# zfkuang/PaletteNeRF

Hardware: AMD Instinct MI355X
Metric: rendered_samples_per_sec (higher is better)
Workload: dtype f32 (field: f16x3 split products, fp32 accumulate); 1 GPU; configs[1]: NeRF-synthetic lego geometry (scene S0), -m nerf inference, 800x800, 1 view(s)/step, camera moving (one pose of the path per step); march_mode=native, fused_field=True, field_precision=f16x3, half_tables=False, ray_order=tile8, frames_in_flight=1, gathered_floats_per_ray=0, rccl_ranks=1, parallelism=single GPU

## Files before the change

### palettenerf_amd/csrc/frame.hip

```cpp
#include "pnr_common.hpp"
#include "march_core.hpp"
#include "grid_core.hpp"
#include "field_core.hpp"
#include "frame_plan.hpp"
#include <hip/hip_ext.h>
#include <vector>
#include <stdlib.h>

uint64_t pnr_internal_edit_device_bytes();
int pnr_internal_edit_upload(const pnr_palette_edit* edit, void* dst, hipStream_t s);
int pnr_internal_palette_field_forward(const pnr_palette_field_args* a, pnr_stream_t stream, int waves12);

#ifndef PNR_FRAME_LEVEL_PAIRS
#define PNR_FRAME_LEVEL_PAIRS 1
#endif
#ifndef PNR_FRAME_LEVEL_PAIRS_PAL
#define PNR_FRAME_LEVEL_PAIRS_PAL 0
#endif
namespace pnr {

struct FrameCtl {
    int32_t n_alive, n_step, step, done;
    int32_t iterations, pad0;
    unsigned long long rendered;
// ... 537 lines not shown
        typedef uint32_t RowT __attribute__((ext_vector_type(NW)));
        __half acc[2 * NT];
#pragma unroll
        for (int ch = 0; ch < 2 * NT; ch++) acc[ch] = __float2half(0.0f);
        if (grid_corner_rows<1>(g, lc, b, idxs, pos)) {
            RowT v[8];
            gather8<RowT, 1, ORDERED>(static_cast<const RowT*>(table) + lc.off0, idxs, v);
            grid_corner_weights(pos, ws);
#pragma unroll
            for (uint32_t idx = 0; idx < 8; idx++) {
                __half hv[2 * NT];
                __builtin_memcpy(hv, &v[idx], sizeof(hv));
#pragma unroll
                for (int ch = 0; ch < 2 * NT; ch++)
                    acc[ch] = __float2half(__half2float(acc[ch]) + __half2float(__float2half(ws[idx] * __half2float(hv[ch]))));
            }
        }
        *reinterpret_cast<float2*>(enc0 + o) = make_float2(__half2float(acc[0]), __half2float(acc[1]));
        if constexpr (NT >= 2) *reinterpret_cast<float2*>(g.enc[1] + o) = make_float2(__half2float(acc[2]), __half2float(acc[3]));
        if constexpr (NT == 3) *reinterpret_cast<float2*>(g.enc[2] + o) = make_float2(__half2float(acc[4]), __half2float(acc[5]));
    }
}

#ifdef PNR_HOSTED_TIMING
__device__ unsigned long long g_hosted_timing[8 + 8 * 256 + 2 * 16 * 128];
__device__ int g_hosted_timing_iter = 3;
#endif
#ifndef PNR_HOSTED_MIN_GLOG
#define PNR_HOSTED_MIN_GLOG 3u
#endif
#ifndef PNR_HOSTED_JUMPS
#define PNR_HOSTED_JUMPS false
#endif
template <int KIND>
__device__ __forceinline__ void hosted_march_tail(const FrameCtl* ctl, const GridArgs& g, const HostedArgs& ha) {
    struct { uint32_t blocks; const int32_t* qctr; const StragglerRec* qrecs; const float* rays_o; const float* rays_d; const uint8_t* bitfield;
             const uint32_t* mip; MarchParams p; float* xyzs; float* dirs; float* deltas; int32_t* partials; } h;
    {
        const HostedConst* hc = ha.hc;
        const int par = ctl->iterations & 1;
        h.blocks = ha.blocks; h.qctr = hc->qctr_all + par * kQueueCtrs; h.qrecs = hc->qrecs; h.rays_o = hc->rays_o; h.rays_d = hc->rays_d;
        h.bitfield = hc->bitfield; h.mip = hc->mip; h.p = hc->p; h.xyzs = hc->xyzs; h.dirs = hc->dirs; h.deltas = hc->deltas;
        h.partials = hc->partials[par] + ha.partial_base;
    }
    __builtin_amdgcn_s_setprio(3);
    __shared__ float lv_scale[16];
// ... 80 lines not shown
            for (uint32_t pi = (uint32_t)lane; pi < cnt * 16u; pi += PNR_WAVE) {
                const uint32_t b = wrows[wave][pi >> 4], level = pi & 15u;
                LevelCtx lc;
                lc.scale = lv_scale[level]; lc.resolution = lv_res[level]; lc.off0 = lv_off[level]; lc.hashmap_size = lv_size[level];
                lc.kind = 0u;
                for (uint32_t tz = 0; tz < n_tab; tz++) grid_row<KIND, false>(g, lc, level, g.table[tz], g.enc[tz], b);
            }
            wave_lds_sync();
        }
    }
    for (int off = PNR_WAVE / 2; off > 0; off >>= 1) emitted += __shfl_xor(emitted, off, PNR_WAVE);
    if (lane == 0) wemit[wave] = emitted;
    __syncthreads();
    if (threadIdx.x == 0) {
        uint32_t tot = 0;
        for (int wv = 0; wv < (int)(kRayBlock / PNR_WAVE); wv++) tot += wemit[wv];
        h.partials[blockIdx.x] = (int32_t)tot;
#ifdef PNR_HOSTED_TIMING
        if (timing) tm[3] = wall_clock64();
#endif
    }
}

template <int KIND>
__device__ __forceinline__ void frame_grid_body(const FrameCtl* __restrict__ ctl, const GridArgs& g, const HostedArgs& h) {
    if (ctl->done) return;
    constexpr uint32_t kLv = KIND == GK_SINGLE ? (PNR_FRAME_LEVEL_PAIRS == 2 ? 4u : (PNR_FRAME_LEVEL_PAIRS ? 2u : 1u))
                                               : ((KIND == GK_PAIR && PNR_FRAME_LEVEL_PAIRS_PAL) ? 2u : 1u);
    constexpr bool kPairs = kLv > 1;
    constexpr uint32_t kNY = 16u / kLv;
    uint32_t bx = blockIdx.x, by = blockIdx.y, bz = blockIdx.z, nbx = gridDim.x;
    if (h.blocks) {
        if (bx < h.blocks) {
#ifndef PNR_NO_HOSTED_CODE
            hosted_march_tail<KIND>(ctl, g, h);
#endif
            return;
        }
        const uint32_t id = bx - h.blocks, yz = id / h.gx;
        bx = id - yz * h.gx; by = yz % kNY; bz = yz / kNY; nbx = h.gx;
    }
    const uint32_t stride = nbx * 256u;
    const uint32_t rows = (uint32_t)ctl->n_alive * (uint32_t)ctl->n_step;
    const uint32_t level = 15u - by;
#ifdef PNR_HOSTED_TIMING
    const bool timing = ctl->iterations == g_hosted_timing_iter && (bx & 15u) == 0 && bx < 2048u && bz == 0;
    unsigned long long* tmm = g_hosted_timing + 8 + 8 * 256 + 2 * (level * 128 + (bx >> 4));
    if (timing && threadIdx.x == 0) tmm[0] = wall_clock64();
#endif
    const LevelCtx lc = level_ctx(g, level);
    [[maybe_unused]] const LevelCtx lc2 = level_ctx(g, kPairs ? by : level);
    [[maybe_unused]] const LevelCtx lc3 = level_ctx(g, kLv == 4 ? 11u - by : level), lc4 = level_ctx(g, kLv == 4 ? 4u + by : level);
    const void* table = g.table[KIND == GK_SINGLE ? bz : 0];
    float* enc0 = g.enc[KIND == GK_SINGLE ? bz : 0];
    for (uint32_t b = bx * 256u + threadIdx.x; b < rows; b += stride) {
        const float d0 = g.deltas[(size_t)b * 2];
        const uint32_t fl = h.rowflag ? h.rowflag[b] : 0u;
        if (d0 == 0.0f || fl) continue;
        grid_row<KIND>(g, lc, level, table, enc0, b);
        if constexpr (kLv == 4) { grid_row<KIND>(g, lc3, 11u - by, table, enc0, b); grid_row<KIND>(g, lc4, 4u + by, table, enc0, b); }
        if constexpr (kPairs) grid_row<KIND>(g, lc2, by, table, enc0, b);
    }
#ifdef PNR_HOSTED_TIMING
    if (timing && threadIdx.x == 0) { asm volatile("s_waitcnt vmcnt(0)" ::: "memory"); tmm[1] = wall_clock64(); }
#endif
}

#ifndef PNR_GRID_WAVES
#define PNR_GRID_WAVES 8
#endif
#ifndef PNR_GRID_WAVES_SINGLE
#define PNR_GRID_WAVES_SINGLE 7
#endif
#define PNR_GRID_KERNEL(NAME, KIND, WAVES)                                                                                                   \
    __global__ void __launch_bounds__(256) __attribute__((amdgpu_waves_per_eu(WAVES))) NAME(const FrameCtl* __restrict__ ctl, GridArgs g, HostedArgs h) { \
        frame_grid_body<KIND>(ctl, g, h);                                                                                                    \
    }
PNR_GRID_KERNEL(k_frame_grid, GK_SINGLE, PNR_GRID_WAVES_SINGLE)
PNR_GRID_KERNEL(k_frame_grid_pair, GK_PAIR, PNR_GRID_WAVES)
PNR_GRID_KERNEL(k_frame_grid_triple, GK_TRIPLE, PNR_GRID_WAVES)
PNR_GRID_KERNEL(k_frame_grid_h1, GK_HALF1, PNR_GRID_WAVES)
PNR_GRID_KERNEL(k_frame_grid_h2, GK_HALF2, PNR_GRID_WAVES)
PNR_GRID_KERNEL(k_frame_grid_h3, GK_HALF3, PNR_GRID_WAVES)
#undef PNR_GRID_KERNEL

__global__ void __launch_bounds__(256) k_interleave_tables(const float2* __restrict__ a, const float2* __restrict__ b, uint64_t rows,
                                                           float4* __restrict__ out) {
    const uint64_t i = (uint64_t)blockIdx.x * 256 + threadIdx.x;
    if (i < rows) { const float2 u = a[i], v = b[i]; out[i] = make_float4(u.x, u.y, v.x, v.y); }
}
__global__ void __launch_bounds__(256) k_interleave_tables3(const float2* __restrict__ a, const float2* __restrict__ b, const float2* __restrict__ c,
                                                            uint64_t rows, float4* __restrict__ out) {
    const uint64_t i = (uint64_t)blockIdx.x * 256 + threadIdx.x;
    if (i < rows) {
        const float2 u = a[i], v = b[i], t = c[i];
        out[2 * i] = make_float4(u.x, u.y, v.x, v.y);
        out[2 * i + 1] = make_float4(t.x, t.y, 0.0f, 0.0f);
    }
}
__global__ void __launch_bounds__(256) k_interleave_tables3_half(const float2* __restrict__ a, const float2* __restrict__ b, const float2* __restrict__ c,
                                                                 uint64_t rows, uint4* __restrict__ out) {
// ... 251 lines not shown
    w.partials[1] = reinterpret_cast<int32_t*>(take((kMaxMarchBlocks + kHostedBlocks) * 4));
    w.enc_pal = w.enc_clip = w.aux = nullptr;
    w.edit = nullptr;
    if (aux_stride) {
        w.edit = take(pnr_internal_edit_device_bytes());
        w.enc_pal = reinterpret_cast<float*>(take(n * 16 * 2 * 4));
        if (with_clip) w.enc_clip = reinterpret_cast<float*>(take(n * 16 * 2 * 4));
        w.aux = reinterpret_cast<float*>(take(n * aux_stride * 4));
    }
    w.s_o = reinterpret_cast<float*>(take(n * 12)); w.s_d = reinterpret_cast<float*>(take(n * 12));
    w.s_noise = reinterpret_cast<float*>(take(n * 4)); w.s_far = reinterpret_cast<float*>(take(n * 4));
    w.s_ws = reinterpret_cast<float*>(take(n * 4)); w.s_depth = reinterpret_cast<float*>(take(n * 4));
    w.s_image = reinterpret_cast<float*>(take(n * 12));
    w.s_aux = aux_stride ? reinterpret_cast<float*>(take(n * aux_stride * 4)) : nullptr;
    w.hosted = reinterpret_cast<HostedConst*>(take(sizeof(HostedConst)));
    w.qctr = reinterpret_cast<int32_t*>(take(2 * kQueueCtrs * 4));
    w.qrecs = reinterpret_cast<StragglerRec*>(take(n * sizeof(StragglerRec)));
    w.rowflag = reinterpret_cast<uint8_t*>(take(n));
    w.bytes = off;
    return w;
}

struct FrameOpts {
    int aux_fusion, composite_fusion, hosted_tail, dynamic_tiles, march_budget, march_budget0, march_blocks, iteration_margin, block_skip, coop_march, palette_waves12;
};
static FrameOpts frame_opts_now() {
    return FrameOpts{g_opt_aux_fusion, g_opt_composite_fusion, g_opt_hosted_tail, g_opt_dynamic_tiles, g_opt_march_budget, g_opt_march_budget0, g_opt_march_blocks,
                     g_opt_iteration_margin, g_opt_block_skip, g_opt_coop_march, g_opt_palette_waves12};
}

using UnsortKernel = decltype(&k_frame_unsort_outputs<4>);
using MarchKernel = decltype(&k_frame_march<true, true, 1>);
using GridKernel = decltype(&k_frame_grid);
using FieldKernel = decltype(&k_frame_field<0, false>);

struct FramePlan {
    pnr_stream_t stream; const void* workspace;
    uint32_t N, max_steps, aux_stride, n_enc, march_lds;
    float T_thresh, density_scale, enc_scale;
    FrameWorkspace w;
    const float *in_o, *in_d, *in_far, *noise_p;
    float *out_ws, *out_depth, *out_image, *out_aux;
    const int32_t* ray_order;
    float *ray_ws, *ray_depth, *ray_image, *ray_aux;
    const uint8_t* bitfield; const uint32_t* mip; const float* packed_weights;
    bool with_clip, half_tables, hosted, use_mip, pow2, pal_composite_fused, timing, has_edit;
    int aux_fused;
    int composite_fused;
    MarchParams mp;
    GridArgs ga;
    pnr_palette_field_args pf;
// ... 77 lines not shown
    p.bitfield = a->bitfield; p.mip = static_cast<const uint32_t*>(a->mip); p.packed_weights = a->packed_weights;
    p.stats = a->stats; p.kernel_ms = a->kernel_ms; p.timing = a->kernel_ms != nullptr;

    p.n_enc = pal ? (p.with_clip ? 3u : 2u) : 1u;
    p.aux_fused = (pal && opt.aux_fusion && pnr_palette_field_stages_aux(pal->num_basis, pal->clip_dim, pal->pred_clip)) ? 1 : 0;
    p.composite_fused = (!pal && opt.composite_fusion) ? opt.composite_fusion : 0;
    p.pal_composite_fused = pal && p.aux_fused && opt.composite_fusion == 2;
    p.half_tables = a->table_dtype == PNR_DTYPE_F16;
    if (p.half_tables && pal && (p.with_clip ? !pal->embeddings_triple : !pal->embeddings_pair)) return PNR_ERR_UNSUPPORTED;
    if (a->table_dtype != PNR_DTYPE_F32 && a->table_dtype != PNR_DTYPE_F16) return PNR_ERR_UNSUPPORTED;

    GridArgs& ga = p.ga;
    ga.xyzs = w.xyzs; ga.deltas = w.deltas; ga.offsets = a->offsets; ga.lp = make_level_params(16, a->S, a->base_resolution); ga.level_stride = p.N;
    ga.bound = a->bound; ga.two_bound = 2.0f * a->bound; ga.inv_two_bound = exact_reciprocal_or_zero(ga.two_bound);
    ga.gridtype = a->gridtype;
    ga.enc[0] = w.enc; ga.enc[1] = w.enc_pal; ga.enc[2] = w.enc_clip;
    p.lookup_y = 16; p.lookup_z = 1;
    if (p.half_tables && pal && p.with_clip) { p.lookup = k_frame_grid_h3; ga.table[0] = pal->embeddings_triple; }
    else if (p.half_tables && pal) { p.lookup = k_frame_grid_h2; ga.table[0] = pal->embeddings_pair; }
    else if (p.half_tables) { p.lookup = k_frame_grid_h1; ga.table[0] = a->embeddings; }
    else if (pal && p.with_clip && pal->embeddings_triple) { p.lookup = k_frame_grid_triple; ga.table[0] = pal->embeddings_triple; }
    else if (pal && !p.with_clip && pal->embeddings_pair) { p.lookup = k_frame_grid_pair; ga.table[0] = pal->embeddings_pair; p.lookup_y = PNR_FRAME_LEVEL_PAIRS_PAL ? 8 : 16; }
    else {
        p.lookup = k_frame_grid; p.lookup_y = PNR_FRAME_LEVEL_PAIRS == 2 ? 4 : (PNR_FRAME_LEVEL_PAIRS ? 8 : 16); p.lookup_z = p.n_enc;
        ga.table[0] = a->embeddings; ga.table[1] = pal ? pal->embeddings_palette : nullptr; ga.table[2] = p.with_clip ? pal->embeddings_clip : nullptr;
    }

    if (pal) {
        pnr_palette_field_args& pf = p.pf;
        pf.enc = w.enc; pf.enc_palette = w.enc_pal; pf.enc_clip = w.enc_clip; pf.level_stride = p.N; pf.dirs = w.dirs; pf.deltas = w.deltas;
        pf.packed = a->packed_weights; pf.num_basis = pal->num_basis;
        pf.clip_dim = pal->clip_dim; pf.pred_clip = pal->pred_clip; pf.density_scale = a->density_scale; pf.offsets_weight = pal->offsets_weight;
        pf.view_dep_weight = pal->view_dep_weight; pf.aux_stride = p.aux_stride; pf.sigmas = w.sigmas; pf.rgbs = w.rgbs; pf.aux = w.aux;
        pf.precision = a->field_precision; pf.xyzs = w.xyzs;
        for (int k = 0; k < 3; k++) pf.enc_scale[k] = a->enc_scale[k];
        pf.overflow_flag = a->watch_overflow ? w.scratch + 1 : nullptr;
        pf.tile_counter = opt.dynamic_tiles ? w.scratch + 2 : nullptr;
        if (p.aux_fused) { pf.weights_sum = p.out_ws; pf.aux_map = p.out_aux; pf.T_thresh = a->T_thresh; }
        if (p.pal_composite_fused) { pf.rays_t = w.rays_t; pf.weights_sum_rw = p.out_ws; pf.depth = p.out_depth; pf.image = p.out_image; }
        if (pal->edit && pal->edit->mode != 0) { p.has_edit = true; p.edit = *pal->edit; pf.edit_device = w.edit; }
    } else {
        p.enc_scale = a->enc_scale[0] > 0.0f ? a->enc_scale[0] : 1.0f;
        p.field = frame_field_kernel(a->field_precision, a->watch_overflow);
    }

    p.use_mip = a->mip && (a->H % 4) == 0 && pnr_occupancy_mip_bytes(a->C, a->H) <= 64 * 1024;
    p.pow2 = is_pow2f(a->bound) && (a->H & (a->H - 1)) == 0;
// ... 248 lines not shown
```

### palettenerf_amd/csrc/grid_core.hpp

```cpp
#pragma once
#include "pnr_common.hpp"
#include <math.h>

namespace pnr {

constexpr uint32_t kMaxLevels = 32;
struct LevelParams {
    float scale[kMaxLevels];
    uint32_t resolution[kMaxLevels];
};

__device__ __forceinline__ float to_f32(float v) { return v; }
__device__ __forceinline__ float to_f32(__half v) { return __half2float(v); }

template <uint32_t D, uint32_t C>
__device__ __forceinline__ uint32_t grid_index(uint32_t gridtype, bool align_corners, uint32_t hashmap_size, uint32_t resolution,
                                               const uint32_t pg[D]) {
    constexpr uint32_t primes[7] = {1u, 2654435761u, 805459861u, 3674653429u, 2097192037u, 1434869437u, 2165219737u};
    uint32_t stride = 1, index = 0;
#pragma unroll
    for (uint32_t d = 0; d < D; d++) {
        if (stride <= hashmap_size) {
            index += pg[d] * stride;
            stride *= align_corners ? resolution : (resolution + 1);
        }
    }
    if (gridtype == 0 && stride > hashmap_size) {
        index = 0;
#pragma unroll
        for (uint32_t d = 0; d < D; d++) index ^= pg[d] * primes[d];
    }
    return (index % hashmap_size) * C;
}

#ifndef PNR_GRID_KIND
#define PNR_GRID_KIND 1
#endif
__device__ __forceinline__ uint32_t level_kind(uint32_t gridtype, uint32_t hashmap_size, uint32_t resolution) {
    if (!PNR_GRID_KIND) return 0u;
    const uint32_t side = resolution + 1u;
    if ((uint64_t)side * side * side <= (uint64_t)hashmap_size) return 1u;
    uint32_t stride = 1u;
#pragma unroll
    for (uint32_t d = 0; d < 3; d++)
        if (stride <= hashmap_size) stride *= side;
    return (gridtype == 0u && stride > hashmap_size && (hashmap_size & (hashmap_size - 1u)) == 0u) ? 2u : 0u;
}
template <uint32_t CMUL>
__device__ __forceinline__ void corner_rows_by_kind(uint32_t kind, uint32_t gridtype, uint32_t hashmap_size, uint32_t resolution, const uint32_t* pg ,
                                                    uint32_t* idxs ) {
    if (kind == 1u) {
        const uint32_t side = resolution + 1u;
#pragma unroll
        for (uint32_t idx = 0; idx < 8; idx++)
            idxs[idx] = ((pg[0] + (idx & 1u)) + (pg[1] + ((idx >> 1) & 1u)) * side + (pg[2] + ((idx >> 2) & 1u)) * side * side) * CMUL;
    } else if (kind == 2u) {
        const uint32_t mask = hashmap_size - 1u;
#pragma unroll
        for (uint32_t idx = 0; idx < 8; idx++)
            idxs[idx] = (((pg[0] + (idx & 1u)) ^ ((pg[1] + ((idx >> 1) & 1u)) * 2654435761u) ^ ((pg[2] + ((idx >> 2) & 1u)) * 805459861u)) & mask) * CMUL;
    } else {
#pragma unroll
        for (uint32_t idx = 0; idx < 8; idx++) {
            uint32_t pl[3];
#pragma unroll
            for (uint32_t d = 0; d < 3; d++) pl[d] = pg[d] + ((idx >> d) & 1u);
            idxs[idx] = grid_index<3, CMUL>(gridtype, false, hashmap_size, resolution, pl);
        }
    }
}
// ... 55 lines not shown
```

### palettenerf_amd/csrc/pnr_common.hpp

```cpp
#pragma once
#include <hip/hip_runtime.h>
#include <hip/hip_fp16.h>
#include <stdint.h>
#include "../../include/pnr.h"

#define PNR_WAVE 64

namespace pnr {

inline int check_launch() {
    hipError_t e = hipGetLastError();
    return e == hipSuccess ? PNR_OK : PNR_ERR_LAUNCH;
}
inline hipStream_t as_stream(pnr_stream_t s) { return reinterpret_cast<hipStream_t>(s); }
inline uint32_t cdiv(uint32_t a, uint32_t b) { return (a + b - 1) / b; }

constexpr int kMaxDevices = 64;
inline int current_device() { int d = 0; if (hipGetDevice(&d) != hipSuccess || d < 0 || d >= kMaxDevices) d = 0; return d; }
template <typename K>
inline bool ensure_dynamic_lds(K kernel, uint32_t bytes, bool* done ) {
    const int d = current_device();
    if (done[d]) return true;
    if (hipFuncSetAttribute(reinterpret_cast<const void*>(kernel), hipFuncAttributeMaxDynamicSharedMemorySize, (int)bytes) != hipSuccess) return false;
    done[d] = true;
// ... 47 lines not shown
    __builtin_amdgcn_sched_barrier(0);
    asm volatile("" :: "v"(p[0]), "v"(p[1]), "v"(p[2]), "v"(p[3]), "v"(p[4]), "v"(p[5]), "v"(p[6]), "v"(p[7]));
}

__device__ __forceinline__ void lds_copy16(const void* gsrc, void* lds) {
    __builtin_amdgcn_global_load_lds((const __attribute__((address_space(1))) void*)gsrc, (__attribute__((address_space(3))) void*)lds, 16, 0, 0);
}
__device__ __forceinline__ void lds_copy_wait() { asm volatile("s_waitcnt vmcnt(0)" ::: "memory"); }
__device__ __forceinline__ uint32_t lds_address(const void* p) { return (uint32_t)reinterpret_cast<uintptr_t>(p); }

__device__ __forceinline__ int wave_inclusive_scan(int v) {
    const int lane = threadIdx.x & (PNR_WAVE - 1);
#pragma unroll
    for (int off = 1; off < PNR_WAVE; off <<= 1) {
        int n = __shfl_up(v, off, PNR_WAVE);
        if (lane >= off) v += n;
    }
    return v;
}

}

extern int g_opt_block_skip;
extern int g_opt_coop_march;
extern int g_opt_hosted_tail;
extern int g_opt_march_budget, g_opt_march_budget0;
extern int g_opt_march_blocks;
extern int g_opt_aux_fusion;
extern int g_opt_composite_fusion;
extern int g_opt_palette_waves12;
extern int g_opt_dynamic_tiles;
extern int g_opt_grid_fast;
extern int g_opt_train_coop;
extern int g_opt_mlp_f16x3;
extern int g_opt_coarse_image;
extern int g_opt_scatter_staged;
extern int g_opt_cell_merge;
extern int g_opt_grid_nt;
extern int g_opt_flex_coop;
extern int g_opt_iteration_margin;
```

### palettenerf_amd/csrc/raymarch.hip

```cpp
#include "pnr_common.hpp"
#include "march_core.hpp"
#include "sph_core.hpp"

namespace pnr {

constexpr uint32_t kBlock = 256;

__global__ void __launch_bounds__(256) k_build_mip(const unsigned long long* __restrict__ grid64, uint32_t nbricks, uint32_t words_per_mask,
                                                   uint32_t* __restrict__ mip) {
    const uint32_t b = blockIdx.x * blockDim.x + threadIdx.x;
    const unsigned long long w = b < nbricks ? grid64[b] : 0ull;
    const unsigned long long any = __ballot(w != 0ull), all = __ballot(b < nbricks && w == ~0ull);
    if ((threadIdx.x & 63) == 0) {
        const uint32_t word = b >> 5;
        if (word < words_per_mask) { mip[word] = (uint32_t)any; mip[words_per_mask + word] = (uint32_t)all; }
        if (word + 1 < words_per_mask) { mip[word + 1] = (uint32_t)(any >> 32); mip[words_per_mask + word + 1] = (uint32_t)(all >> 32); }
    }
}


__global__ void __launch_bounds__(kBlock) k_near_far(const float* __restrict__ rays_o, const float* __restrict__ rays_d,
                                                     const float* __restrict__ aabb, uint32_t N, float min_near,
                                                     float* __restrict__ nears, float* __restrict__ fars) {
    const uint32_t n = blockIdx.x * kBlock + threadIdx.x;
// ... 448 lines not shown
    const float* P = poses + (size_t)b * 16;
    float* o = rays_o + ((size_t)b * N + n) * 3;
    float* d = rays_d + ((size_t)b * N + n) * 3;
#pragma unroll
    for (int k = 0; k < 3; k++) {
        d[k] = fmaf(d2, P[k * 4 + 2], fmaf(d1, P[k * 4 + 1], d0 * P[k * 4 + 0]));
        o[k] = P[k * 4 + 3];
    }
}

}

int g_opt_block_skip = getenv("PNR_NO_BLOCK_SKIP") ? 0 : 1;
int g_opt_coop_march = getenv("PNR_NO_COOP_MARCH") ? 0 : 1;
int g_opt_hosted_tail = getenv("PNR_NO_HOSTED_TAIL") ? 0 : 1;
int g_opt_march_budget = getenv("PNR_MARCH_BUDGET") ? atoi(getenv("PNR_MARCH_BUDGET")) : 2;
int g_opt_march_budget0 = getenv("PNR_MARCH_BUDGET0") ? atoi(getenv("PNR_MARCH_BUDGET0")) : 0;
int g_opt_march_blocks = getenv("PNR_MARCH_BLOCKS") ? atoi(getenv("PNR_MARCH_BLOCKS")) : 0;
int g_opt_aux_fusion = getenv("PNR_NO_AUX_FUSION") ? 0 : 1;
int g_opt_composite_fusion = getenv("PNR_NO_COMPOSITE_FUSION") ? 0 : (getenv("PNR_COMPOSITE_FUSION") ? atoi(getenv("PNR_COMPOSITE_FUSION")) : 2);
int g_opt_iteration_margin = getenv("PNR_ITERATION_MARGIN") ? atoi(getenv("PNR_ITERATION_MARGIN")) : 0;
int g_opt_palette_waves12 = getenv("PNR_PALETTE_WAVES8") ? 0 : 1;
int g_opt_dynamic_tiles = getenv("PNR_DYNAMIC_TILES") ? 1 : 0;
int g_opt_grid_fast = getenv("PNR_NO_GRID_FAST") ? 0 : 1;
int g_opt_train_coop = getenv("PNR_NO_TRAIN_COOP") ? 0 : 1;
int g_opt_mlp_f16x3 = getenv("PNR_MLP_FP32") ? 0 : 1;
int g_opt_coarse_image = getenv("PNR_NO_COARSE_IMAGE") ? 0 : 1;
int g_opt_scatter_staged = getenv("PNR_NO_SCATTER_STAGED") ? 0 : 1;
int g_opt_cell_merge = getenv("PNR_NO_CELL_MERGE") ? 0 : 1;
int g_opt_flex_coop = getenv("PNR_NO_FLEX_COOP") ? 0 : 1;
int g_opt_grid_nt = getenv("PNR_GRID_NT") ? atoi(getenv("PNR_GRID_NT")) : 0;
int g_opt_adam_variant = 0;

using namespace pnr;

extern "C" {

int pnr_abi_version(void) { return 10; }

int pnr_set_option(const char* name, int value) {
    if (!name) return PNR_ERR_INVALID;
    if (!strcmp(name, "block_skip")) { g_opt_block_skip = value != 0; return PNR_OK; }
    if (!strcmp(name, "coop_march")) { g_opt_coop_march = value != 0; return PNR_OK; }
    if (!strcmp(name, "hosted_tail")) { g_opt_hosted_tail = value != 0; return PNR_OK; }
    if (!strcmp(name, "march_budget")) { g_opt_march_budget = value < 1 ? 1 : (value > 1024 ? 1024 : value); return PNR_OK; }
    if (!strcmp(name, "march_budget0")) { g_opt_march_budget0 = value < 0 ? 0 : (value > 1024 ? 1024 : value); return PNR_OK; }
    if (!strcmp(name, "march_blocks")) { g_opt_march_blocks = value < 0 ? 0 : value; return PNR_OK; }
    if (!strcmp(name, "aux_fusion")) { g_opt_aux_fusion = value != 0; return PNR_OK; }
    if (!strcmp(name, "composite_fusion")) { g_opt_composite_fusion = value < 0 ? 0 : (value > 2 ? 2 : value); return PNR_OK; }
    if (!strcmp(name, "palette_waves12")) { g_opt_palette_waves12 = value != 0; return PNR_OK; }
    if (!strcmp(name, "dynamic_tiles")) { g_opt_dynamic_tiles = value != 0; return PNR_OK; }
    if (!strcmp(name, "grid_fast")) { g_opt_grid_fast = value != 0; return PNR_OK; }
    if (!strcmp(name, "train_coop")) { g_opt_train_coop = value != 0; return PNR_OK; }
    if (!strcmp(name, "mlp_f16x3")) { g_opt_mlp_f16x3 = value != 0; return PNR_OK; }
    if (!strcmp(name, "coarse_image")) { g_opt_coarse_image = value != 0; return PNR_OK; }
    if (!strcmp(name, "cell_merge")) { g_opt_cell_merge = value != 0; return PNR_OK; }
    if (!strcmp(name, "scatter_staged")) { g_opt_scatter_staged = value != 0; return PNR_OK; }
    if (!strcmp(name, "flex_coop")) { g_opt_flex_coop = value != 0; return PNR_OK; }
    if (!strcmp(name, "grid_nt")) { g_opt_grid_nt = value & 3; return PNR_OK; }
    if (!strcmp(name, "adam_variant")) { g_opt_adam_variant = value & 7; return PNR_OK; }
    if (!strcmp(name, "iteration_margin")) { g_opt_iteration_margin = value < 0 ? 0 : (value > 64 ? 64 : value); return PNR_OK; }
    return PNR_ERR_INVALID;
}

const char* pnr_error_string(int code) {
    switch (code) {
        case PNR_OK: return "ok";
        case PNR_ERR_INVALID: return "invalid argument (null pointer or bad size)";
        case PNR_ERR_UNSUPPORTED: return "unsupported configuration";
        case PNR_ERR_LAUNCH: return "HIP kernel launch failed";
        case PNR_ERR_ALIGNMENT: return "an activation array does not start on a 16-byte boundary or holds fewer than four floats (pnr_mlp_* move tiles as 16-byte requests: copy such a view)";
        default: return "unknown error";
    }
}
// ... 201 lines not shown
```

### profiles/micro/gather_rate.hip

```cpp
#include <hip/hip_runtime.h>
#include <stdint.h>
#include <stdio.h>
#include <vector>

template <typename T> __device__ __forceinline__ float first(const T& v);
template <> __device__ __forceinline__ float first<float>(const float& v) { return v; }
template <> __device__ __forceinline__ float first<float2>(const float2& v) { return v.x + v.y; }
template <> __device__ __forceinline__ float first<float4>(const float4& v) { return v.x + v.y + v.z + v.w; }

template <typename T, int UNROLL, bool PAIR>
__global__ void __launch_bounds__(256) k(const T* __restrict__ table, uint32_t mask, uint32_t loads_per_lane, uint32_t seed, float* __restrict__ out) {
    uint32_t s = (blockIdx.x * 256 + threadIdx.x) * 2654435761u + seed;
    float acc = 0.0f;
    for (uint32_t i = 0; i < loads_per_lane; i += UNROLL) {
        T v[UNROLL];
#pragma unroll
        for (int u = 0; u < UNROLL; u++) {
            s = s * 1664525u + 1013904223u;
            uint32_t r = (s >> 4) & mask;
            if (PAIR && (u & 1)) r = (((s - 1013904223u) * 4000846301u >> 4) & mask) ^ 1u;
            v[u] = table[r];
        }
#pragma unroll
        for (int u = 0; u < UNROLL; u++) acc += first<T>(v[u]);
    }
    if (acc == 123.456f) out[0] = acc;
}

template <typename T, bool PAIR>
void run(const char* name, const void* table, size_t table_bytes, float* out) {
    const uint32_t rows = (uint32_t)(table_bytes / sizeof(T));
    uint32_t mask = 1; while ((mask << 1) <= rows) mask <<= 1; mask -= 1;
    const uint32_t blocks = 256 * 8, loads = 256;
    hipEvent_t e0, e1;
    (void)hipEventCreate(&e0); (void)hipEventCreate(&e1);
    hipLaunchKernelGGL((k<T, 8, PAIR>), dim3(blocks), dim3(256), 0, 0, (const T*)table, mask, loads, 1u, out);
    (void)hipEventRecord(e0);
    const int reps = 5;
    for (int i = 0; i < reps; i++) hipLaunchKernelGGL((k<T, 8, PAIR>), dim3(blocks), dim3(256), 0, 0, (const T*)table, mask, loads, 7u + i, out);
    (void)hipEventRecord(e1);
    (void)hipEventSynchronize(e1);
    float ms; (void)hipEventElapsedTime(&ms, e0, e1);
    const double lane_loads = (double)blocks * 256 * loads * reps;
    const double sec = ms * 1e-3;
    printf("%-34s table %6.0f MB: %7.1f G lane-loads/s = %5.2f per clock per CU, %7.1f GB/s useful\n", name, table_bytes / 1048576.0, lane_loads / sec / 1e9,
           lane_loads / sec / (256 * 2.4e9), lane_loads * sizeof(T) / sec / 1e9);
}

int main() {
    const size_t big = 512ull << 20;
    void* table; float* out;
    (void)hipMalloc(&table, big); (void)hipMalloc(&out, 64);
    (void)hipMemset(table, 0, big);
    for (size_t mb : {4ull, 50ull, 512ull}) {
        const size_t bytes = mb << 20;
        run<float, false>("4-byte rows (half2 row)", table, bytes, out);
        run<float2, false>("8-byte rows (fp32 row)", table, bytes, out);
        run<float2, true>("8-byte rows, every 2nd adjacent", table, bytes, out);
        run<float4, false>("16-byte rows (two tables interleaved)", table, bytes, out);
    }
    return 0;
}
```

Measured before the change: 3.081 billion samples/s.

## Split hash-grid corner gathers across lane pairs for fine levels

Adds a lane-pair path for the single-table grid lookup kernel on levels at or above a threshold. Adjacent lanes exchange grid coordinates through DPP swaps, and each lane fetches one x-side of the cube (four corners) for both samples, so the two x-neighbour corners that sit next to each other in memory come from the same cache line within a pair. Rows are then swapped back with DPP before accumulation. It is enabled by default through a new option and adds cross-lane shuffles, branching on the validity of the partner lane, and separate handling for out-of-bound samples.

```diff
diff --git a/palettenerf_amd/csrc/frame.hip b/palettenerf_amd/csrc/frame.hip
--- a/palettenerf_amd/csrc/frame.hip
+++ b/palettenerf_amd/csrc/frame.hip
@@ -583,6 +583,134 @@
     }
 }
 
+__device__ __forceinline__ uint32_t dpp_swap_pair(uint32_t x) { return (uint32_t)__builtin_amdgcn_update_dpp(0, (int)x, 0xB1 , 0xF, 0xF, true); }
+template <int KIND>
+__device__ __forceinline__ void grid_pair_level(const GridArgs& g, const LevelCtx& lc, uint32_t level, const void* __restrict__ table, float* __restrict__ enc0, uint32_t b,
+                                                const float (&in)[3], bool live, bool ok, bool odd, bool okA, bool okB) {
+    static_assert(KIND == GK_SINGLE, "the one-table fp32 layout");
+    constexpr int NW = 2;
+    typedef f32x2 RowT;
+    float pos[3];
+    uint32_t pg[3], ag[3], bg[3];
+#pragma unroll
+    for (int d = 0; d < 3; d++) {
+        pos[d] = fmaf(in[d], lc.scale, 0.5f);
+        const float fl = floorf(pos[d]);
+        pg[d] = (uint32_t)fl;
+        pos[d] -= (float)pg[d];
+        const uint32_t qg = dpp_swap_pair(pg[d]);
+        ag[d] = odd ? qg : pg[d];
+        bg[d] = odd ? pg[d] : qg;
+    }
+    uint32_t idxs[8];
+    x_side_rows<1>(lc.kind, g.gridtype, lc.hashmap_size, lc.resolution, ag, odd ? 1u : 0u, idxs);
+    x_side_rows<1>(lc.kind, g.gridtype, lc.hashmap_size, lc.resolution, bg, odd ? 1u : 0u, idxs + 4);
+    const RowT* tab = static_cast<const RowT*>(table) + lc.off0;
+    const RowT* p[8];
+#pragma unroll
+    for (int i = 0; i < 8; i++) p[i] = tab + idxs[i];
+    RowT v[8] = {};
+    if (okA && okB) load8_fresh(p, v);
+    else if (okA) {
+#pragma unroll
+        for (int i = 0; i < 4; i++) v[i] = *(typename GlobalPtr<RowT>::type)(uintptr_t)p[i];
+    } else {
+#pragma unroll
+        for (int i = 4; i < 8; i++) v[i] = *(typename GlobalPtr<RowT>::type)(uintptr_t)p[i];
+    }
+    float ws[8];
+    grid_corner_weights(pos, ws);
+    uint32_t cw[8][NW];
+#pragma unroll
+    for (int jk = 0; jk < 4; jk++) {
+        uint32_t wa[NW], wb[NW];
+        __builtin_memcpy(wa, &v[jk], sizeof(wa));
+        __builtin_memcpy(wb, &v[4 + jk], sizeof(wb));
+#pragma unroll
+        for (int w = 0; w < NW; w++) {
+            const uint32_t sa = dpp_swap_pair(wa[w]), sb = dpp_swap_pair(wb[w]);
+            cw[2 * jk][w] = odd ? sb : wa[w];
+            cw[2 * jk + 1][w] = odd ? wb[w] : sa;
+        }
+    }
+    const size_t o = ((size_t)level * g.level_stride + b) * 2;
+    float acc[2] = {0.0f, 0.0f};
+#pragma unroll
+    for (uint32_t idx = 0; idx < 8; idx++) {
+        acc[0] = fmaf(ws[idx], __builtin_bit_cast(float, cw[idx][0]), acc[0]);
+        acc[1] = fmaf(ws[idx], __builtin_bit_cast(float, cw[idx][1]), acc[1]);
+    }
+    const float2 out = make_float2(acc[0], acc[1]);
+    if (ok) *reinterpret_cast<float2*>(enc0 + o) = out;
+    else if (live) *reinterpret_cast<float2*>(enc0 + o) = make_float2(0.0f, 0.0f);
+}
+template <int KIND>
+__device__ __forceinline__ void grid_row_at(const GridArgs& g, const LevelCtx& lc, uint32_t level, const void* __restrict__ table, float* __restrict__ enc0, uint32_t b,
+                                            const float (&in)[3]) {
+    static_assert(KIND == GK_SINGLE, "the one-table fp32 layout");
+    float pos[3], ws[8];
+    uint32_t pg[3], idxs[8];
+#pragma unroll
+    for (int d = 0; d < 3; d++) {
+        pos[d] = fmaf(in[d], lc.scale, 0.5f);
+        const float fl = floorf(pos[d]);
+        pg[d] = (uint32_t)fl;
+        pos[d] -= (float)pg[d];
+    }
+    corner_rows_by_kind<1>(lc.kind, g.gridtype, lc.hashmap_size, lc.resolution, pg, idxs);
+    f32x2 v[8];
+    gather8<f32x2, 1, true>(static_cast<const f32x2*>(table) + lc.off0, idxs, v);
+    grid_corner_weights(pos, ws);
+    float acc[2] = {0.0f, 0.0f};
+#pragma unroll
+    for (uint32_t idx = 0; idx < 8; idx++) { acc[0] = fmaf(ws[idx], v[idx].x, acc[0]); acc[1] = fmaf(ws[idx], v[idx].y, acc[1]); }
+    *reinterpret_cast<float2*>(enc0 + ((size_t)level * g.level_stride + b) * 2) = make_float2(acc[0], acc[1]);
+}
+template <int KIND, uint32_t NLV>
+__device__ __forceinline__ void grid_pair_rows(const GridArgs& g, const LevelCtx (&lcs)[NLV], const uint32_t (&levels)[NLV], const void* __restrict__ table, float* __restrict__ enc0,
+                                               const uint8_t* __restrict__ rowflag, uint32_t first, uint32_t stride, uint32_t rows) {
+    const bool odd = (threadIdx.x & 1u) != 0;
+    for (uint32_t b = first; (b & ~1u) < rows; b += stride) {
+        bool live = false, ok = false;
+        float in[3] = {0.0f, 0.0f, 0.0f};
+        if (b < rows) {
+            const float d0 = g.deltas[(size_t)b * 2];
+            const uint32_t fl = rowflag ? rowflag[b] : 0u;
+            live = d0 != 0.0f && !fl;
+        }
+        if (live) {
+            float xyz[3];
+#pragma unroll
+            for (int d = 0; d < 3; d++) xyz[d] = g.xyzs[(size_t)b * 3 + d];
+            asm volatile("" : "+v"(xyz[0]), "+v"(xyz[1]), "+v"(xyz[2]));
+            bool oob = false;
+#pragma unroll
+            for (int d = 0; d < 3; d++) {
+                const float sft = xyz[d] + g.bound;
+                in[d] = g.inv_two_bound != 0.0f ? sft * g.inv_two_bound : sft / g.two_bound;
+                oob |= (in[d] < 0.0f) | (in[d] > 1.0f);
+            }
+            ok = !oob;
+            if (oob) { in[0] = 0.0f; in[1] = 0.0f; in[2] = 0.0f; }
+        }
+        const bool pok = dpp_swap_pair(ok ? 1u : 0u) != 0u;
+        const bool okA = odd ? pok : ok, okB = odd ? ok : pok;
+        if (!(okA || okB)) {
+            if (live) {
+#pragma unroll
+                for (uint32_t l = 0; l < NLV; l++) *reinterpret_cast<float2*>(enc0 + ((size_t)levels[l] * g.level_stride + b) * 2) = make_float2(0.0f, 0.0f);
+            }
+            continue;
+        }
+        grid_pair_level<KIND>(g, lcs[0], levels[0], table, enc0, b, in, live, ok, odd, okA, okB);
+#pragma unroll
+        for (uint32_t l = 1; l < NLV; l++) {
+            if (ok) grid_row_at<KIND>(g, lcs[l], levels[l], table, enc0, b, in);
+            else if (live) *reinterpret_cast<float2*>(enc0 + ((size_t)levels[l] * g.level_stride + b) * 2) = make_float2(0.0f, 0.0f);
+        }
+    }
+}
+
 #ifdef PNR_HOSTED_TIMING
 __device__ unsigned long long g_hosted_timing[8 + 8 * 256 + 2 * 16 * 128];
 __device__ int g_hosted_timing_iter = 3;
@@ -709,7 +837,10 @@
     }
 }
 
-template <int KIND>
+#ifndef PNR_LANE_PAIR_MIN_LEVEL
+#define PNR_LANE_PAIR_MIN_LEVEL 8u
+#endif
+template <int KIND, bool LANE_PAIRS = false>
 __device__ __forceinline__ void frame_grid_body(const FrameCtl* __restrict__ ctl, const GridArgs& g, const HostedArgs& h) {
     if (ctl->done) return;
     constexpr uint32_t kLv = KIND == GK_SINGLE ? (PNR_FRAME_LEVEL_PAIRS == 2 ? 4u : (PNR_FRAME_LEVEL_PAIRS ? 2u : 1u))
@@ -740,6 +871,23 @@
     [[maybe_unused]] const LevelCtx lc3 = level_ctx(g, kLv == 4 ? 11u - by : level), lc4 = level_ctx(g, kLv == 4 ? 4u + by : level);
     const void* table = g.table[KIND == GK_SINGLE ? bz : 0];
     float* enc0 = g.enc[KIND == GK_SINGLE ? bz : 0];
+    bool paired = false;
+    if constexpr (LANE_PAIRS) {
+        static_assert(kLv <= 2, "one or two levels per workgroup row");
+        if (level >= PNR_LANE_PAIR_MIN_LEVEL) {
+            paired = true;
+            if constexpr (kPairs) {
+                const LevelCtx lcs[2] = {lc, lc2};
+                const uint32_t levels[2] = {level, by};
+                grid_pair_rows<KIND, 2>(g, lcs, levels, table, enc0, h.rowflag, bx * 256u + threadIdx.x, stride, rows);
+            } else {
+                const LevelCtx lcs[1] = {lc};
+                const uint32_t levels[1] = {level};
+                grid_pair_rows<KIND, 1>(g, lcs, levels, table, enc0, h.rowflag, bx * 256u + threadIdx.x, stride, rows);
+            }
+        }
+    }
+    if (!paired)
     for (uint32_t b = bx * 256u + threadIdx.x; b < rows; b += stride) {
         const float d0 = g.deltas[(size_t)b * 2];
         const uint32_t fl = h.rowflag ? h.rowflag[b] : 0u;
@@ -759,11 +907,12 @@
 #ifndef PNR_GRID_WAVES_SINGLE
 #define PNR_GRID_WAVES_SINGLE 7
 #endif
-#define PNR_GRID_KERNEL(NAME, KIND, WAVES)                                                                                                   \
+#define PNR_GRID_KERNEL(NAME, KIND, WAVES, ...)                                                                                              \
     __global__ void __launch_bounds__(256) __attribute__((amdgpu_waves_per_eu(WAVES))) NAME(const FrameCtl* __restrict__ ctl, GridArgs g, HostedArgs h) { \
-        frame_grid_body<KIND>(ctl, g, h);                                                                                                    \
+        frame_grid_body<KIND, ##__VA_ARGS__>(ctl, g, h);                                                                                     \
     }
 PNR_GRID_KERNEL(k_frame_grid, GK_SINGLE, PNR_GRID_WAVES_SINGLE)
+PNR_GRID_KERNEL(k_frame_grid_lp, GK_SINGLE, PNR_GRID_WAVES_SINGLE, true)
 PNR_GRID_KERNEL(k_frame_grid_pair, GK_PAIR, PNR_GRID_WAVES)
 PNR_GRID_KERNEL(k_frame_grid_triple, GK_TRIPLE, PNR_GRID_WAVES)
 PNR_GRID_KERNEL(k_frame_grid_h1, GK_HALF1, PNR_GRID_WAVES)
@@ -1061,11 +1210,11 @@
 }
 
 struct FrameOpts {
-    int aux_fusion, composite_fusion, hosted_tail, dynamic_tiles, march_budget, march_budget0, march_blocks, iteration_margin, block_skip, coop_march, palette_waves12;
+    int aux_fusion, composite_fusion, hosted_tail, dynamic_tiles, march_budget, march_budget0, march_blocks, iteration_margin, block_skip, coop_march, palette_waves12, grid_lane_pairs;
 };
 static FrameOpts frame_opts_now() {
     return FrameOpts{g_opt_aux_fusion, g_opt_composite_fusion, g_opt_hosted_tail, g_opt_dynamic_tiles, g_opt_march_budget, g_opt_march_budget0, g_opt_march_blocks,
-                     g_opt_iteration_margin, g_opt_block_skip, g_opt_coop_march, g_opt_palette_waves12};
+                     g_opt_iteration_margin, g_opt_block_skip, g_opt_coop_march, g_opt_palette_waves12, g_opt_grid_lane_pairs};
 }
 
 using UnsortKernel = decltype(&k_frame_unsort_outputs<4>);
@@ -1189,7 +1338,7 @@
     else if (pal && p.with_clip && pal->embeddings_triple) { p.lookup = k_frame_grid_triple; ga.table[0] = pal->embeddings_triple; }
     else if (pal && !p.with_clip && pal->embeddings_pair) { p.lookup = k_frame_grid_pair; ga.table[0] = pal->embeddings_pair; p.lookup_y = PNR_FRAME_LEVEL_PAIRS_PAL ? 8 : 16; }
     else {
-        p.lookup = k_frame_grid; p.lookup_y = PNR_FRAME_LEVEL_PAIRS == 2 ? 4 : (PNR_FRAME_LEVEL_PAIRS ? 8 : 16); p.lookup_z = p.n_enc;
+        p.lookup = opt.grid_lane_pairs ? k_frame_grid_lp : k_frame_grid; p.lookup_y = PNR_FRAME_LEVEL_PAIRS == 2 ? 4 : (PNR_FRAME_LEVEL_PAIRS ? 8 : 16); p.lookup_z = p.n_enc;
         ga.table[0] = a->embeddings; ga.table[1] = pal ? pal->embeddings_palette : nullptr; ga.table[2] = p.with_clip ? pal->embeddings_clip : nullptr;
     }
 
diff --git a/palettenerf_amd/csrc/grid_core.hpp b/palettenerf_amd/csrc/grid_core.hpp
--- a/palettenerf_amd/csrc/grid_core.hpp
+++ b/palettenerf_amd/csrc/grid_core.hpp
@@ -1,5 +1,6 @@
 #pragma once
 #include "pnr_common.hpp"
+#include "grid_xside.hpp"
 #include <math.h>
 
 namespace pnr {
@@ -33,19 +34,6 @@
     return (index % hashmap_size) * C;
 }
 
-#ifndef PNR_GRID_KIND
-#define PNR_GRID_KIND 1
-#endif
-__device__ __forceinline__ uint32_t level_kind(uint32_t gridtype, uint32_t hashmap_size, uint32_t resolution) {
-    if (!PNR_GRID_KIND) return 0u;
-    const uint32_t side = resolution + 1u;
-    if ((uint64_t)side * side * side <= (uint64_t)hashmap_size) return 1u;
-    uint32_t stride = 1u;
-#pragma unroll
-    for (uint32_t d = 0; d < 3; d++)
-        if (stride <= hashmap_size) stride *= side;
-    return (gridtype == 0u && stride > hashmap_size && (hashmap_size & (hashmap_size - 1u)) == 0u) ? 2u : 0u;
-}
 template <uint32_t CMUL>
 __device__ __forceinline__ void corner_rows_by_kind(uint32_t kind, uint32_t gridtype, uint32_t hashmap_size, uint32_t resolution, const uint32_t* pg ,
                                                     uint32_t* idxs ) {
diff --git a/palettenerf_amd/csrc/grid_xside.hpp b/palettenerf_amd/csrc/grid_xside.hpp
--- /dev/null
+++ b/palettenerf_amd/csrc/grid_xside.hpp
@@ -0,0 +1,67 @@
+#pragma once
+#include <stdint.h>
+
+#ifndef PNR_HD
+#if defined(__HIPCC__)
+#define PNR_HD __host__ __device__ __forceinline__
+#else
+#define PNR_HD inline
+#endif
+#endif
+
+namespace pnr {
+
+#ifndef PNR_GRID_KIND
+#define PNR_GRID_KIND 1
+#endif
+PNR_HD uint32_t level_kind(uint32_t gridtype, uint32_t hashmap_size, uint32_t resolution) {
+    if (!PNR_GRID_KIND) return 0u;
+    const uint32_t side = resolution + 1u;
+    if ((uint64_t)side * side * side <= (uint64_t)hashmap_size) return 1u;
+    uint32_t stride = 1u;
+    for (uint32_t d = 0; d < 3; d++)
+        if (stride <= hashmap_size) stride *= side;
+    return (gridtype == 0u && stride > hashmap_size && (hashmap_size & (hashmap_size - 1u)) == 0u) ? 2u : 0u;
+}
+
+template <uint32_t CMUL>
+PNR_HD uint32_t grid_index3(uint32_t gridtype, uint32_t hashmap_size, uint32_t resolution, const uint32_t* pl ) {
+    uint32_t stride = 1, index = 0;
+    for (uint32_t d = 0; d < 3; d++) {
+        if (stride <= hashmap_size) {
+            index += pl[d] * stride;
+            stride *= resolution + 1u;
+        }
+    }
+    if (gridtype == 0 && stride > hashmap_size) index = pl[0] ^ (pl[1] * 2654435761u) ^ (pl[2] * 805459861u);
+    return (index % hashmap_size) * CMUL;
+}
+
+template <uint32_t CMUL>
+PNR_HD void x_side_rows(uint32_t kind, uint32_t gridtype, uint32_t hashmap_size, uint32_t resolution, const uint32_t* pg , uint32_t xside,
+                        uint32_t* rows ) {
+    const uint32_t x = pg[0] + xside;
+    if (kind == 1u) {
+        const uint32_t side = resolution + 1u;
+#if defined(__HIPCC__)
+#pragma unroll
+#endif
+        for (uint32_t jk = 0; jk < 4; jk++) rows[jk] = (x + (pg[1] + (jk & 1u)) * side + (pg[2] + (jk >> 1)) * side * side) * CMUL;
+    } else if (kind == 2u) {
+        const uint32_t mask = hashmap_size - 1u;
+#if defined(__HIPCC__)
+#pragma unroll
+#endif
+        for (uint32_t jk = 0; jk < 4; jk++) rows[jk] = ((x ^ ((pg[1] + (jk & 1u)) * 2654435761u) ^ ((pg[2] + (jk >> 1)) * 805459861u)) & mask) * CMUL;
+    } else {
+#if defined(__HIPCC__)
+#pragma unroll
+#endif
+        for (uint32_t jk = 0; jk < 4; jk++) {
+            const uint32_t pl[3] = {x, pg[1] + (jk & 1u), pg[2] + (jk >> 1)};
+            rows[jk] = grid_index3<CMUL>(gridtype, hashmap_size, resolution, pl);
+        }
+    }
+}
+
+}
diff --git a/palettenerf_amd/csrc/pnr_common.hpp b/palettenerf_amd/csrc/pnr_common.hpp
--- a/palettenerf_amd/csrc/pnr_common.hpp
+++ b/palettenerf_amd/csrc/pnr_common.hpp
@@ -93,6 +93,7 @@
 }
 
 extern int g_opt_block_skip;
+extern int g_opt_grid_lane_pairs;
 extern int g_opt_coop_march;
 extern int g_opt_hosted_tail;
 extern int g_opt_march_budget, g_opt_march_budget0;
diff --git a/palettenerf_amd/csrc/raymarch.hip b/palettenerf_amd/csrc/raymarch.hip
--- a/palettenerf_amd/csrc/raymarch.hip
+++ b/palettenerf_amd/csrc/raymarch.hip
@@ -494,6 +494,7 @@
 int g_opt_iteration_margin = getenv("PNR_ITERATION_MARGIN") ? atoi(getenv("PNR_ITERATION_MARGIN")) : 0;
 int g_opt_palette_waves12 = getenv("PNR_PALETTE_WAVES8") ? 0 : 1;
 int g_opt_dynamic_tiles = getenv("PNR_DYNAMIC_TILES") ? 1 : 0;
+int g_opt_grid_lane_pairs = getenv("PNR_GRID_LANE_PAIRS") ? atoi(getenv("PNR_GRID_LANE_PAIRS")) != 0 : 1;
 int g_opt_grid_fast = getenv("PNR_NO_GRID_FAST") ? 0 : 1;
 int g_opt_train_coop = getenv("PNR_NO_TRAIN_COOP") ? 0 : 1;
 int g_opt_mlp_f16x3 = getenv("PNR_MLP_FP32") ? 0 : 1;
@@ -522,6 +523,7 @@
     if (!strcmp(name, "composite_fusion")) { g_opt_composite_fusion = value < 0 ? 0 : (value > 2 ? 2 : value); return PNR_OK; }
     if (!strcmp(name, "palette_waves12")) { g_opt_palette_waves12 = value != 0; return PNR_OK; }
     if (!strcmp(name, "dynamic_tiles")) { g_opt_dynamic_tiles = value != 0; return PNR_OK; }
+    if (!strcmp(name, "grid_lane_pairs")) { g_opt_grid_lane_pairs = value != 0; return PNR_OK; }
     if (!strcmp(name, "grid_fast")) { g_opt_grid_fast = value != 0; return PNR_OK; }
     if (!strcmp(name, "train_coop")) { g_opt_train_coop = value != 0; return PNR_OK; }
     if (!strcmp(name, "mlp_f16x3")) { g_opt_mlp_f16x3 = value != 0; return PNR_OK; }
diff --git a/profiles/grid_line_sharing.py b/profiles/grid_line_sharing.py
--- /dev/null
+++ b/profiles/grid_line_sharing.py
@@ -0,0 +1,138 @@
+import argparse
+import os
+import sys
+
+import numpy as np
+import torch
+
+ROOT = os.path.dirname(os.path.dirname(os.path.abspath(__file__)))
+sys.path.insert(0, ROOT)
+
+LINE = 128
+ROW_BYTES = 8
+_P1, _P2, _M32 = 2654435761, 805459861, 0xFFFFFFFF
+
+
+def record_positions(crop, iterations):
+    import bench
+    import oracle
+    from oracle.facade import make_oracle_modules
+    from palettenerf_amd import renderer, scene
+    from palettenerf_amd.fused import tile_ray_order
+    import palettenerf_amd.gridencoder as pge
+    import palettenerf_amd.shencoder as psh
+    args = bench.parse(["--workload", "lego"])
+    H, W = args.wl["H"], args.wl["W"]
+    pose = torch.from_numpy(bench.pose_of(args, 0)[None])
+    ro, rd = scene.get_rays(pose, bench.intrinsics_of(args), H, W)
+    idx = bench.crop_indices(H, W, crop)
+    idx = idx[tile_ray_order(torch.arange(crop * crop), crop, 8).long()]
+    ro, rd = ro[:, idx].contiguous(), rd[:, idx].contiguous()
+    rm, ge, sh, _ = make_oracle_modules()
+    seen, calls = {}, [0]
+    inner = rm.march_rays
+
+    def march_rays(n_alive, n_step, *a, **k):
+        x, d, dl = inner(n_alive, n_step, *a, **k)
+        if calls[0] in iterations:
+            rows = n_alive * n_step
+            seen[calls[0]] = (x[:rows].numpy().copy(), dl[:rows, 0].numpy() != 0, n_step)
+        calls[0] += 1
+        return x, d, dl
+
+    rm.march_rays = march_rays
+    saved = (renderer.raymarching, pge.GridEncoder, psh.SHEncoder)
+    renderer.raymarching, pge.GridEncoder, psh.SHEncoder = rm, ge.GridEncoder, sh.SHEncoder
+    try:
+        m = bench.make_model(args, "nerf")
+        scene.seed_field_(m, 0)
+        grid = bench.density_grid_of(args.wl["scene"])
+        m.density_grid.copy_(torch.from_numpy(grid))
+        m.density_bitfield.copy_(torch.from_numpy(oracle.packbits(grid, 0.5)))
+        m.eval()
+        with torch.no_grad():
+            m.render(ro, rd, perturb=False, dt_gamma=args.wl["dt_gamma"], max_steps=1024, T_thresh=1e-4)
+        bound, enc = float(m.bound), m.encoder
+        offs = [int(o) for o in enc.offsets.tolist()]
+        scale, res = oracle.grid_level_params(len(offs) - 1, enc.per_level_scale, enc.base_resolution)
+    finally:
+        renderer.raymarching, pge.GridEncoder, psh.SHEncoder = saved
+    out = {}
+    for it, (x, live, n_step) in seen.items():
+        out[it] = ((x + bound) / (2 * bound), live, n_step)
+    return out, offs, [float(s) for s in scale], [int(r) for r in res], calls[0]
+
+
+def corner_lines(x, offs, scale, res, lv):
+    size, side = offs[lv + 1] - offs[lv], res[lv] + 1
+    pos = x.astype(np.float32) * np.float32(scale[lv]) + np.float32(0.5)
+    pg = np.floor(pos).astype(np.int64).clip(min=0)
+    dense = side ** 3 <= size
+    lines = np.empty((x.shape[0], 8), np.int64)
+    for c in range(8):
+        p = [pg[:, d] + ((c >> d) & 1) for d in range(3)]
+        if dense:
+            index = p[0] + p[1] * side + p[2] * (side * side)
+        else:
+            index = (p[0] & _M32) ^ ((p[1] * _P1) & _M32) ^ ((p[2] * _P2) & _M32)
+        lines[:, c] = ((offs[lv] + index % size) * ROW_BYTES) // LINE
+    return lines
+
+
+def per_instruction(lines_by_lane):
+    v = lines_by_lane[lines_by_lane >= 0]
+    quads = 0
+    for q in range(0, 64, 4):
+        s = lines_by_lane[q:q + 4]
+        quads += len(set(s[s >= 0].tolist()))
+    return len(set(v.tolist())), quads
+
+
+def count(lines, live):
+    rows = lines.shape[0]
+    pad = (-rows) % 64
+    lines = np.concatenate([lines, np.full((pad, 8), -1, np.int64)])
+    live = np.concatenate([live, np.zeros(pad, bool)])
+    lines[~live] = -1
+    tot = np.zeros(5)
+    n_waves = 0
+    for w0 in range(0, lines.shape[0], 64):
+        wl = lines[w0:w0 + 64]
+        if not (wl >= 0).any():
+            continue
+        n_waves += 1
+        for c in range(8):
+            a, b = per_instruction(wl[:, c])
+            tot[0] += a; tot[3] += b
+        for half in range(2):
+            for jk in range(4):
+                by_lane = np.empty(64, np.int64)
+                by_lane[0::2] = wl[half::2, 2 * jk]
+                by_lane[1::2] = wl[half::2, 2 * jk + 1]
+                a, b = per_instruction(by_lane)
+                tot[1] += a; tot[4] += b
+        tot[2] += len(set(wl[wl >= 0].tolist()))
+    return tot / max(n_waves, 1), n_waves
+
+
+def main():
+    ap = argparse.ArgumentParser()
+    ap.add_argument("--crop", type=int, default=128)
+    ap.add_argument("--iterations", type=int, nargs="*", default=[0, 5, 15, 25])
+    a = ap.parse_args()
+    seen, offs, scale, res, n_iter = record_positions(a.crop, set(a.iterations))
+    print(f"# lego pose 0, centre {a.crop}x{a.crop}, 8x8 tile order; the oracle's loop ran {n_iter} iterations; lines of {LINE} bytes, rows of {ROW_BYTES}")
+    for it in sorted(seen):
+        x, live, n_step = seen[it]
+        print(f"\niteration {it}: {x.shape[0]} rows (n_step {n_step}), {live.mean() * 100:.1f} % live")
+        print(f"{'level':>5} {'lane = sample':>14} {'lane pair':>10} {'whole wave':>11} {'quad cycles':>12} {'pair quad cycles':>17}")
+        sums = np.zeros(5)
+        for lv in range(len(offs) - 1):
+            t, _ = count(corner_lines(x, offs, scale, res, lv), live)
+            sums += t
+            print(f"{lv:5d} {t[0]:14.1f} {t[1]:10.1f} {t[2]:11.1f} {t[3]:12.1f} {t[4]:17.1f}")
+        print(f"  all {sums[0]:14.1f} {sums[1]:10.1f} {sums[2]:11.1f} {sums[3]:12.1f} {sums[4]:17.1f}    pair / today: {sums[1] / sums[0]:.2f} in lines, {sums[4] / sums[3]:.2f} in quad cycles")
+
+
+if __name__ == "__main__":
+    main()
diff --git a/profiles/micro/gather_rate.hip b/profiles/micro/gather_rate.hip
--- a/profiles/micro/gather_rate.hip
+++ b/profiles/micro/gather_rate.hip
@@ -8,9 +8,10 @@
 template <> __device__ __forceinline__ float first<float2>(const float2& v) { return v.x + v.y; }
 template <> __device__ __forceinline__ float first<float4>(const float4& v) { return v.x + v.y + v.z + v.w; }
 
-template <typename T, int UNROLL, bool PAIR>
+template <typename T, int UNROLL, bool PAIR, bool LANEPAIR = false>
 __global__ void __launch_bounds__(256) k(const T* __restrict__ table, uint32_t mask, uint32_t loads_per_lane, uint32_t seed, float* __restrict__ out) {
-    uint32_t s = (blockIdx.x * 256 + threadIdx.x) * 2654435761u + seed;
+    const uint32_t tid = blockIdx.x * 256 + threadIdx.x;
+    uint32_t s = (LANEPAIR ? tid >> 1 : tid) * 2654435761u + seed;
     float acc = 0.0f;
     for (uint32_t i = 0; i < loads_per_lane; i += UNROLL) {
         T v[UNROLL];
@@ -19,6 +20,7 @@
             s = s * 1664525u + 1013904223u;
             uint32_t r = (s >> 4) & mask;
             if (PAIR && (u & 1)) r = (((s - 1013904223u) * 4000846301u >> 4) & mask) ^ 1u;
+            if (LANEPAIR) r ^= tid & 1u;
             v[u] = table[r];
         }
 #pragma unroll
@@ -27,17 +29,17 @@
     if (acc == 123.456f) out[0] = acc;
 }
 
-template <typename T, bool PAIR>
+template <typename T, bool PAIR, bool LANEPAIR = false>
 void run(const char* name, const void* table, size_t table_bytes, float* out) {
     const uint32_t rows = (uint32_t)(table_bytes / sizeof(T));
     uint32_t mask = 1; while ((mask << 1) <= rows) mask <<= 1; mask -= 1;
     const uint32_t blocks = 256 * 8, loads = 256;
     hipEvent_t e0, e1;
     (void)hipEventCreate(&e0); (void)hipEventCreate(&e1);
-    hipLaunchKernelGGL((k<T, 8, PAIR>), dim3(blocks), dim3(256), 0, 0, (const T*)table, mask, loads, 1u, out);
+    hipLaunchKernelGGL((k<T, 8, PAIR, LANEPAIR>), dim3(blocks), dim3(256), 0, 0, (const T*)table, mask, loads, 1u, out);
     (void)hipEventRecord(e0);
     const int reps = 5;
-    for (int i = 0; i < reps; i++) hipLaunchKernelGGL((k<T, 8, PAIR>), dim3(blocks), dim3(256), 0, 0, (const T*)table, mask, loads, 7u + i, out);
+    for (int i = 0; i < reps; i++) hipLaunchKernelGGL((k<T, 8, PAIR, LANEPAIR>), dim3(blocks), dim3(256), 0, 0, (const T*)table, mask, loads, 7u + i, out);
     (void)hipEventRecord(e1);
     (void)hipEventSynchronize(e1);
     float ms; (void)hipEventElapsedTime(&ms, e0, e1);
@@ -58,6 +60,8 @@
         run<float2, false>("8-byte rows (fp32 row)", table, bytes, out);
         run<float2, true>("8-byte rows, every 2nd adjacent", table, bytes, out);
         run<float4, false>("16-byte rows (two tables interleaved)", table, bytes, out);
+        run<float2, false, true>("lane pair r, r^1: 8-byte rows", table, bytes, out);
+        run<float, false, true>("lane pair r, r^1: 4-byte rows", table, bytes, out);
     }
     return 0;
 }
```

New measurement: 3.185 billion samples/s (median of 6 runs). 1.03x the previous value.
